# llm-d/llm-d-workload-variant-autoscaler

Hardware: AMD Instinct MI355X
Metric: desired-replica accuracy + SLO-attainment %, Llama-3-8B synthetic QPS ramp (higher is better)
Workload: dtype bf16; 1 GPU; model=meta-llama/Llama-3.1-8B, global_batch=256, seq_len=150, parallelism=dp1, device=AMD Radeon Graphics

## Files before the change

### wva_amd/calibration/model.py

```python
from __future__ import annotations

import math
from dataclasses import dataclass
from typing import List, Optional

import torch

from .. import ops


@dataclass
class LlamaConfig:
    name: str = "llama"
    hidden_size: int = 4096
    intermediate_size: int = 14336
    num_layers: int = 32
    num_q_heads: int = 32
    num_kv_heads: int = 8
    head_dim: int = 128
    vocab_size: int = 128256
    rope_theta: float = 500000.0
    rms_eps: float = 1e-5

    @property
# ... 146 lines not shown
            if self.cache_dtype == torch.bfloat16:
                self.k_cache[layer][:batch, :, :context_len].normal_(0.0, 1.0)
                self.v_cache[layer][:batch, :, :context_len].normal_(0.0, 1.0)
            else:
                shape = self.k_cache[layer][:batch, :, :context_len].shape
                for cache in (self.k_cache, self.v_cache):
                    cache[layer][:batch, :, :context_len] = torch.randn(
                        shape, device=self.device, dtype=torch.bfloat16
                    ).to(self.cache_dtype)

    def _linear(self, x: torch.Tensor, layer, name: str) -> torch.Tensor:
        if self.weights_dtype == "bf16":
            w = getattr(layer, name) if layer is not None else self.lm_head
            return ops.linear(x, w)
        w8, w_scale = (
            getattr(layer, name + "_q") if layer is not None else self.lm_head_q
        )
        if not x.is_cuda:
            return (
                x.float() @ (w8.float() * w_scale[:, None]).t()
            ).to(x.dtype)
        if x.shape[0] <= 64 and x.shape[1] % 128 == 0:
            from .. import ops as _ops

            return _ops._require_ext().skinny_linear_fp8(x, w8, w_scale)
        return (x @ (w8.to(x.dtype) * w_scale[:, None].to(x.dtype)).t())

    @torch.no_grad()
    def decode_step(self, token_ids: torch.Tensor) -> torch.Tensor:
        cfg = self.cfg
        B = token_ids.shape[0]
        positions = self.context_lens[:B].clone()

        ctx = positions + 1
        x = self.embed.index_select(0, token_ids)
        residual: Optional[torch.Tensor] = None

        for li, layer in enumerate(self.layers):
            if residual is None:
                residual = x.clone()
                h = ops.rmsnorm(x, layer.input_norm, None, cfg.rms_eps)
            else:
                h = ops.rmsnorm(x, layer.input_norm, residual, cfg.rms_eps)

            qkv = self._linear(h, layer, "wqkv")
            q = ops.rope_append_kv(
                qkv, self.k_cache[li][:B], self.v_cache[li][:B],
                positions, cfg.num_q_heads, cfg.num_kv_heads, cfg.rope_theta,
            )

            attn = ops.gqa_decode_attn(
                q, self.k_cache[li][:B], self.v_cache[li][:B], ctx, self.scale
            )
            x = self._linear(attn.reshape(B, cfg.q_size), layer, "wo")

            h2 = ops.rmsnorm(x, layer.post_attn_norm, residual, cfg.rms_eps)
            gate_up = self._linear(h2, layer, "w_gate_up")
            act = ops.silu_mul_fused(gate_up)
            x = self._linear(act, layer, "w_down")

        final = ops.rmsnorm(x, self.final_norm, residual, cfg.rms_eps)
        logits = self._linear(final, None, "lm_head")
        self.context_lens[:B] += 1
        return logits

    @torch.no_grad()
    def prefill(self, token_ids: torch.Tensor) -> torch.Tensor:
        cfg = self.cfg
        if self.weights_dtype != "bf16":
            raise NotImplementedError(
                "prefill with fp8 weights is not implemented (the "
                "weight-only fp8 mode targets decode; prefill would "
                "dequantize every layer per pass)"
            )
        B, S = token_ids.shape
        T = B * S
        if S > self.max_seq:
            raise ValueError(f"S={S} exceeds max_seq={self.max_seq}")
        positions = (
            torch.arange(S, device=self.device, dtype=torch.int32)
            .repeat(B)
        )

        x = self.embed.index_select(0, token_ids.reshape(-1))
        residual: Optional[torch.Tensor] = None
# ... 74 lines not shown
```

### wva_amd/calibration/moe_model.py

```python
from __future__ import annotations

import math
from dataclasses import dataclass
from typing import List, Optional

import torch

from .. import ops


@dataclass
class MixtralConfig:
    name: str = "mistralai/Mixtral-8x7B"
    hidden_size: int = 4096
    intermediate_size: int = 14336
    num_layers: int = 32
    num_q_heads: int = 32
    num_kv_heads: int = 8
    head_dim: int = 128
    vocab_size: int = 32000
    rope_theta: float = 1000000.0
    rms_eps: float = 1e-5
    num_experts: int = 8
    top_k: int = 2
# ... 178 lines not shown
        cfg = self.cfg
        B = h2.shape[0]
        E, I = cfg.num_experts, cfg.intermediate_size
        w_full = torch.zeros(B, E, device=h2.device, dtype=h2.dtype)
        w_full.scatter_(1, selected, weights)
        gate_up = ops.linear(h2, layer.w_gate_up_flat)
        act = ops.silu_mul_fused(
            gate_up.reshape(B * E, 2 * I)
        ).reshape(B, E, I)
        y = torch.bmm(act.transpose(0, 1).contiguous(), layer.w_down_t)
        return (y * w_full.t().unsqueeze(-1)).sum(dim=0)

    def _moe_mlp_sparse(self, layer, h2, weights, selected):
        cfg = self.cfg
        out = torch.zeros_like(h2)
        for e in range(cfg.num_experts):
            mask = selected == e
            token_idx, k_idx = mask.nonzero(as_tuple=True)
            if token_idx.numel() == 0:
                continue
            x_e = h2.index_select(0, token_idx)
            gate_up = ops.linear(x_e, layer.w_gate_up[e])
            act = ops.silu_mul_fused(gate_up)
            y = ops.linear(act, layer.w_down[e])
            w_e = weights[token_idx, k_idx].unsqueeze(-1)
            out.index_add_(0, token_idx, (y * w_e).to(out.dtype))
        return out

    @torch.no_grad()
    def decode_step(self, token_ids: torch.Tensor) -> torch.Tensor:
        cfg = self.cfg
        B = token_ids.shape[0]
        positions = self.context_lens[:B].clone()
        ctx = positions + 1

        x = self.embed.index_select(0, token_ids)
        residual: Optional[torch.Tensor] = None

        for li, layer in enumerate(self.layers):
            if residual is None:
                residual = x.clone()
                h = ops.rmsnorm(x, layer.input_norm, None, cfg.rms_eps)
            else:
                h = ops.rmsnorm(x, layer.input_norm, residual, cfg.rms_eps)

            qkv = ops.linear(h, layer.wqkv)
            q = ops.rope_append_kv(
                qkv, self.k_cache[li][:B], self.v_cache[li][:B],
                positions, cfg.num_q_heads, cfg.num_kv_heads, cfg.rope_theta,
            )
            attn = ops.gqa_decode_attn(
                q, self.k_cache[li][:B], self.v_cache[li][:B], ctx, self.scale
            )
            x = ops.linear(attn.reshape(B, cfg.q_size), layer.wo)

            h2 = ops.rmsnorm(x, layer.post_attn_norm, residual, cfg.rms_eps)
            x = self._moe_mlp(layer, h2)

        final = ops.rmsnorm(x, self.final_norm, residual, cfg.rms_eps)
        logits = ops.linear(final, self.lm_head)
        self.context_lens[:B] += 1
        return logits

    @torch.no_grad()
    def prefill(self, token_ids: torch.Tensor) -> torch.Tensor:
        cfg = self.cfg
        B, S = token_ids.shape
        T = B * S
        if S > self.max_seq:
            raise ValueError(f"S={S} exceeds max_seq={self.max_seq}")
        positions = (
            torch.arange(S, device=self.device, dtype=torch.int32).repeat(B)
        )

        x = self.embed.index_select(0, token_ids.reshape(-1))
        residual = None
        causal = None
        if not x.is_cuda:
            causal = torch.full(
                (S, S), float("-inf"), device=self.device, dtype=torch.float32
            ).triu(1)

        for li, layer in enumerate(self.layers):
            if residual is None:
                residual = x.clone()
# ... 60 lines not shown
```

### wva_amd/calibration/tp_model.py

```python
from __future__ import annotations

import math
from typing import List, Optional

import torch
import torch.distributed as dist

from .. import ops
from .model import LlamaConfig


class _TPLayer:
    def __init__(self, cfg: LlamaConfig, shard: "TPShardInfo", device, dtype, gen):
        h, std = cfg.hidden_size, 0.02

        def w(rows, cols):
            return torch.empty(rows, cols, device=device, dtype=dtype).normal_(
                0.0, std, generator=gen
            )

        self.input_norm = torch.ones(h, device=device, dtype=dtype)
        self.post_attn_norm = torch.ones(h, device=device, dtype=dtype)
        self.wqkv = w(shard.q_size + 2 * shard.kv_size, h)
        self.wo = w(h, shard.q_size)
# ... 72 lines not shown
        self.v_cache = [
            torch.zeros_like(self.k_cache[0]) for _ in range(cfg.num_layers)
        ]
        self.context_lens = torch.zeros(
            max_batch, dtype=torch.int32, device=self.device
        )
        self.scale = 1.0 / math.sqrt(cfg.head_dim)

    def _all_reduce(self, x: torch.Tensor) -> torch.Tensor:
        if self.tp > 1:
            dist.all_reduce(x, group=self.group)
        return x

    def reset(self, batch: int, context_len: int) -> None:
        self.context_lens.zero_()
        self.context_lens[:batch] = context_len
        for layer in range(self.cfg.num_layers):
            if self.cache_dtype == torch.bfloat16:
                self.k_cache[layer][:batch, :, :context_len].normal_(0.0, 1.0)
                self.v_cache[layer][:batch, :, :context_len].normal_(0.0, 1.0)
            else:
                shape = self.k_cache[layer][:batch, :, :context_len].shape
                for cache in (self.k_cache, self.v_cache):
                    cache[layer][:batch, :, :context_len] = torch.randn(
                        shape, device=self.device, dtype=torch.bfloat16
                    ).to(self.cache_dtype)

    @torch.no_grad()
    def decode_step(self, token_ids: torch.Tensor) -> torch.Tensor:
        cfg, shard = self.cfg, self.shard
        B = token_ids.shape[0]
        positions = self.context_lens[:B].clone()

        ctx = positions + 1
        x = self.embed.index_select(0, token_ids)
        residual: Optional[torch.Tensor] = None

        for li, layer in enumerate(self.layers):
            if residual is None:
                residual = x.clone()
                h = ops.rmsnorm(x, layer.input_norm, None, cfg.rms_eps)
            else:
                h = ops.rmsnorm(x, layer.input_norm, residual, cfg.rms_eps)

            qkv = ops.linear(h, layer.wqkv)
            q = ops.rope_append_kv(
                qkv, self.k_cache[li][:B], self.v_cache[li][:B],
                positions, shard.num_q_heads, shard.num_kv_heads,
                cfg.rope_theta,
            )
            attn = ops.gqa_decode_attn(
                q, self.k_cache[li][:B], self.v_cache[li][:B], ctx, self.scale
            )
            x = self._all_reduce(ops.linear(attn.reshape(B, shard.q_size), layer.wo))

            h2 = ops.rmsnorm(x, layer.post_attn_norm, residual, cfg.rms_eps)
            gate_up = ops.linear(h2, layer.w_gate_up)
            act = ops.silu_mul_fused(gate_up)
            x = self._all_reduce(ops.linear(act, layer.w_down))

        final = ops.rmsnorm(x, self.final_norm, residual, cfg.rms_eps)
        logits = ops.linear(final, self.lm_head)
        self.context_lens[:B] += 1
        return logits
```

### wva_amd/ops/__init__.py

```python
from __future__ import annotations

import glob
import importlib.util
import math
import os
from typing import Optional

import torch

_HERE = os.path.dirname(os.path.abspath(__file__))
_ext = None
_ext_error: Optional[str] = None


def _try_load_extension():
    global _ext, _ext_error
    if _ext is not None:
        return _ext
    candidates = sorted(glob.glob(os.path.join(_HERE, "_wva_ops*.so")))
    if not candidates:
        _ext_error = (
            f"HIP extension _wva_ops*.so not found in {_HERE}; build it with "
            "`python -m wva_amd.ops.build` (or __graft_entry__.build())"
        )
# ... 228 lines not shown
    idx = torch.arange(B)
    k_cache[idx, :, positions.long()] = k.to(k_cache.dtype)
    v_cache[idx, :, positions.long()] = v.to(v_cache.dtype)
    return q


def silu_mul_fused(gate_up: torch.Tensor) -> torch.Tensor:
    if gate_up.is_cuda:
        return _require_ext().silu_mul_fused(gate_up)
    inter = gate_up.shape[1] // 2
    return silu_mul_ref(gate_up[:, :inter], gate_up[:, inter:]).to(
        gate_up.dtype
    )


def gqa_decode_attn(
    q: torch.Tensor,
    k_cache: torch.Tensor,
    v_cache: torch.Tensor,
    context_lens: torch.Tensor,
    scale: Optional[float] = None,
) -> torch.Tensor:
    if scale is None:
        scale = 1.0 / math.sqrt(q.shape[-1])
    if q.is_cuda:
        return _require_ext().gqa_decode_attn(
            q, k_cache, v_cache, context_lens.to(torch.int32), scale
        )
    return gqa_decode_attn_ref(q, k_cache, v_cache, context_lens, scale).to(
        q.dtype
    )


def moe_route(router_logits: torch.Tensor, top_k: int):
    if router_logits.is_cuda:
        return tuple(
            _require_ext().moe_route(
                router_logits.float().contiguous(), top_k
            )
        )
    return moe_route_ref(router_logits, top_k)


def moe_gate_up_swiglu(
    x: torch.Tensor,
    w_gate_up: torch.Tensor,
    expert_offsets: torch.Tensor,
    sorted_slots: torch.Tensor,
    top_k: int,
) -> torch.Tensor:
    if x.is_cuda:
        return _require_ext().moe_gate_up_swiglu(
            x, w_gate_up, expert_offsets, sorted_slots, top_k
        )
    return moe_gate_up_swiglu_ref(
        x, w_gate_up, expert_offsets, sorted_slots, top_k
    ).to(x.dtype)


def moe_down_combine(
    act_sorted: torch.Tensor,
    w_down: torch.Tensor,
    topk_w: torch.Tensor,
    expert_offsets: torch.Tensor,
    sorted_slots: torch.Tensor,
) -> torch.Tensor:
# ... 71 lines not shown
```

### wva_amd/ops/csrc/attention.hip

```cpp
#include "common.h"

#include <type_traits>

#define HEAD_DIM 128
#define MAX_G 8
#define TILE 64
#define NUM_WAVES 4
#define ROW_DW 66
#define S_ROW 65

template <bool KV_FP8>
using kv_elem_t = std::conditional_t<KV_FP8, fp8_t, bf16>;

__device__ __forceinline__ long ws_row_offset(int b, int kvh, int g, int split,
                                              int num_kv_heads, int G,
                                              int num_splits) {
  return ((((long)b * num_kv_heads + kvh) * G + g) * num_splits + split) *
         (2 + HEAD_DIM);
}

__device__ __forceinline__ long pack8_fp8(const float* v, float inv_scale) {
  unsigned int lo = 0, hi = 0;
  lo = __builtin_amdgcn_cvt_pk_fp8_f32(v[0] * inv_scale, v[1] * inv_scale,
                                       lo, false);
  lo = __builtin_amdgcn_cvt_pk_fp8_f32(v[2] * inv_scale, v[3] * inv_scale,
                                       lo, true);
  hi = __builtin_amdgcn_cvt_pk_fp8_f32(v[4] * inv_scale, v[5] * inv_scale,
                                       hi, false);
  hi = __builtin_amdgcn_cvt_pk_fp8_f32(v[6] * inv_scale, v[7] * inv_scale,
                                       hi, true);
  return (long)(((unsigned long)hi << 32) | lo);
}

struct QFrags {
  bf16x8_frag bf[4];
  long fp8[4];
  float scale;
};

template <bool KV_FP8>
__device__ __forceinline__ QFrags load_q_frags(const bf16* __restrict__ q,
                                               int b, int kvh, int G,
                                               int num_q_heads, int lane,
                                               int wave, int g, int k0,
                                               float* qmax_lds) {
  QFrags qf;
  qf.scale = 1.0f;
#pragma unroll
  for (int kk = 0; kk < 4; ++kk) qf.fp8[kk] = 0;
  float qv[4][8];
#pragma unroll
  for (int kk = 0; kk < 4; ++kk)
#pragma unroll
    for (int i = 0; i < 8; ++i) qv[kk][i] = 0.0f;
  if (g < G) {
    const bf16* qrow = q + ((long)b * num_q_heads + kvh * G + g) * HEAD_DIM;
#pragma unroll
    for (int kk = 0; kk < 4; ++kk) {
      const short* src = reinterpret_cast<const short*>(qrow + 32 * kk + k0);
#pragma unroll
      for (int i = 0; i < 8; ++i) {
        qf.bf[kk][i] = src[i];
        const bf16 bv = *reinterpret_cast<const bf16*>(&src[i]);
        qv[kk][i] = bf2f(bv);
      }
    }
  } else {
#pragma unroll
    for (int kk = 0; kk < 4; ++kk)
#pragma unroll
      for (int i = 0; i < 8; ++i) qf.bf[kk][i] = 0;
  }
  if constexpr (KV_FP8) {
    float amax = 0.0f;
#pragma unroll
    for (int kk = 0; kk < 4; ++kk)
#pragma unroll
      for (int i = 0; i < 8; ++i) amax = fmaxf(amax, fabsf(qv[kk][i]));
    amax = wave_reduce_max(amax);
    if (lane == 0) qmax_lds[wave] = amax;
    __syncthreads();
    float m0 = qmax_lds[0];
#pragma unroll
    for (int w2 = 1; w2 < NUM_WAVES; ++w2) m0 = fmaxf(m0, qmax_lds[w2]);
    qf.scale = fmaxf(m0 / 448.0f, 1e-12f);
    const float inv = 1.0f / qf.scale;
#pragma unroll
    for (int kk = 0; kk < 4; ++kk) qf.fp8[kk] = pack8_fp8(qv[kk], inv);
    __syncthreads();
  }
  return qf;
}

struct SoftmaxStep {
  float p;
  float corr;
};

__device__ __forceinline__ SoftmaxStep online_softmax_step(
    const float* __restrict__ s_row, int tn, int lane, float& m, float& s) {
  const bool live = lane < tn;
  const float score = live ? s_row[lane] : -INFINITY;
  const float tile_max = wave_reduce_max(score);
  const float m_new = fmaxf(m, tile_max);
  const float p = live ? __expf(score - m_new) : 0.0f;
  const float tile_sum = wave_reduce_sum(p);
  const float corr = (m == -INFINITY) ? 0.0f : __expf(m - m_new);
  s = s * corr + tile_sum;
  m = m_new;
  return {p, corr};
}

template <bool KV_FP8>
__global__ __launch_bounds__(256, 2) void gqa_decode_attn_v4_kernel(
    bf16* __restrict__ out,
    float* __restrict__ workspace,
    const bf16* __restrict__ q,
    const void* __restrict__ k_cache,
    const void* __restrict__ v_cache,
    const int* __restrict__ context_lens,
    const int num_q_heads,
    const int num_kv_heads,
    const int max_seq,
    const float scale) {
  const int b = blockIdx.x;
  const int kvh = blockIdx.y;
  const int split = blockIdx.z;
  const int num_splits = gridDim.z;
  const int G = num_q_heads / num_kv_heads;
  const int ctx = context_lens[b];

  const int lane = threadIdx.x & (WAVE_SIZE - 1);
  const int wave = threadIdx.x / WAVE_SIZE;
  const int frag_col = lane % 16;
  const int frag_k0 = 8 * (lane / 16);

  __shared__ float s_smem[MAX_G][S_ROW];
  __shared__ unsigned int v_smem[TILE * ROW_DW];
  __shared__ float p_smem[MAX_G][TILE];
  float* qmax_lds = nullptr;
  if constexpr (KV_FP8) {
    __shared__ float qmax_smem[NUM_WAVES];
    qmax_lds = qmax_smem;
  }

  const QFrags qf = load_q_frags<KV_FP8>(q, b, kvh, G, num_q_heads, lane,
                                         wave, frag_col, frag_k0, qmax_lds);

  const int heads_mine = (G > wave) ? (G - wave + NUM_WAVES - 1) / NUM_WAVES : 0;
  float m[2], s[2], acc[2][2];
#pragma unroll
  for (int j = 0; j < 2; ++j) {
    m[j] = -INFINITY;
    s[j] = 0.0f;
    acc[j][0] = acc[j][1] = 0.0f;
  }

  const long slab_off = ((long)b * num_kv_heads + kvh) * max_seq * HEAD_DIM;
  const auto* k_slab =
      reinterpret_cast<const kv_elem_t<KV_FP8>*>(k_cache) + slab_off;
  const auto* v_slab =
      reinterpret_cast<const kv_elem_t<KV_FP8>*>(v_cache) + slab_off;

  for (int t0 = split * TILE; t0 < ctx; t0 += num_splits * TILE) {
    const int tn = min(TILE, ctx - t0);

    if constexpr (KV_FP8) {
      const int tile_g8 = tn * (HEAD_DIM / 8);
      const fp8_t* v_src = v_slab + (long)t0 * HEAD_DIM;
      for (int idx = wave * WAVE_SIZE + lane; idx < tile_g8;
           idx += NUM_WAVES * WAVE_SIZE) {
        const int row = idx >> 4;
        const int d8 = (idx & 15) * 8;
        const unsigned short* src =
            reinterpret_cast<const unsigned short*>(
                v_src + (long)row * HEAD_DIM + d8);
        unsigned int* dst = &v_smem[row * ROW_DW + d8 / 2];
#pragma unroll
        for (int j = 0; j < 4; ++j) {
          const float2_vt f = unpk2_fp8(src[j]);
// ... 73 lines not shown
        const float p = pg[t];
        a0 = fmaf(p, bf2f(vv.x), a0);
        a1 = fmaf(p, bf2f(vv.y), a1);
      }
      acc[j][0] = a0;
      acc[j][1] = a1;
    }
    __syncthreads();
  }

  if (num_splits == 1) {
    for (int j = 0; j < heads_mine; ++j) {
      const int g = wave + j * NUM_WAVES;
      const float inv = s[j] > 0.0f ? 1.0f / s[j] : 0.0f;
      bf16x2* orow = reinterpret_cast<bf16x2*>(
          out + ((long)b * num_q_heads + kvh * G + g) * HEAD_DIM);
      orow[lane] = bf16x2{f2bf(acc[j][0] * inv), f2bf(acc[j][1] * inv)};
    }
  } else {
    for (int j = 0; j < heads_mine; ++j) {
      const int g = wave + j * NUM_WAVES;
      float* wsp = workspace +
          ws_row_offset(b, kvh, g, split, num_kv_heads, G, num_splits);
      if (lane == 0) {
        wsp[0] = m[j];
        wsp[1] = s[j];
      }
      wsp[2 + 2 * lane] = acc[j][0];
      wsp[2 + 2 * lane + 1] = acc[j][1];
    }
  }
}

template <bool KV_FP8>
__global__ __launch_bounds__(256, 2) void gqa_decode_attn_v5_kernel(
    bf16* __restrict__ out,
    float* __restrict__ workspace,
    const bf16* __restrict__ q,
    const void* __restrict__ k_cache,
    const void* __restrict__ v_cache,
    const int* __restrict__ context_lens,
    const int num_q_heads,
    const int num_kv_heads,
    const int max_seq,
    const float scale) {
  const int b = blockIdx.x;
  const int kvh = blockIdx.y;
  const int split = blockIdx.z;
  const int num_splits = gridDim.z;
  const int G = num_q_heads / num_kv_heads;
  const int ctx = context_lens[b];

  const int lane = threadIdx.x & (WAVE_SIZE - 1);
  const int wave = threadIdx.x / WAVE_SIZE;
  const int frag_col = lane % 16;
  const int frag_k0 = 8 * (lane / 16);

  __shared__ float s_smem[MAX_G][S_ROW];
  __shared__ unsigned int v_smem[TILE * ROW_DW];
  __shared__ float p_smem[MAX_G][TILE];
  __shared__ float corr_smem[MAX_G];
  __shared__ float sum_smem[MAX_G];
  __shared__ float m_smem[MAX_G];
  float* qmax_lds = nullptr;
  if constexpr (KV_FP8) {
    __shared__ float qmax_smem[NUM_WAVES];
    qmax_lds = qmax_smem;
  }

  const QFrags qf = load_q_frags<KV_FP8>(q, b, kvh, G, num_q_heads, lane,
                                         wave, frag_col, frag_k0, qmax_lds);

  const int heads_mine = (G > wave) ? (G - wave + NUM_WAVES - 1) / NUM_WAVES : 0;
  float m[2], s[2];
#pragma unroll
  for (int j = 0; j < 2; ++j) {
    m[j] = -INFINITY;
    s[j] = 0.0f;
  }
  f32x4_frag acc_pv[2] = {f32x4_frag{0.f, 0.f, 0.f, 0.f},
                          f32x4_frag{0.f, 0.f, 0.f, 0.f}};

  const long slab_off = ((long)b * num_kv_heads + kvh) * max_seq * HEAD_DIM;
  const auto* k_slab =
      reinterpret_cast<const kv_elem_t<KV_FP8>*>(k_cache) + slab_off;
  const auto* v_slab =
      reinterpret_cast<const kv_elem_t<KV_FP8>*>(v_cache) + slab_off;

  for (int t0 = split * TILE; t0 < ctx; t0 += num_splits * TILE) {
    const int tn = min(TILE, ctx - t0);

    if constexpr (KV_FP8) {
      const int tile_g8 = tn * (HEAD_DIM / 8);
      const fp8_t* v_src = v_slab + (long)t0 * HEAD_DIM;
      for (int idx = wave * WAVE_SIZE + lane; idx < tile_g8;
           idx += NUM_WAVES * WAVE_SIZE) {
        const int row = idx >> 4;
        const int d8 = (idx & 15) * 8;
        const unsigned short* src =
            reinterpret_cast<const unsigned short*>(
                v_src + (long)row * HEAD_DIM + d8);
        unsigned int* dst = &v_smem[row * ROW_DW + d8 / 2];
#pragma unroll
        for (int j = 0; j < 4; ++j) {
// ... 205 lines not shown
    if (sm_m[w] == -INFINITY) continue;
    const float f = __expf(sm_m[w] - Mg);
    Sg += sm_s[w] * f;
    g0 = fmaf(sm_o[w][2 * lane], f, g0);
    g1 = fmaf(sm_o[w][2 * lane + 1], f, g1);
  }
  const float inv = Sg > 0.0f ? 1.0f / Sg : 0.0f;
  bf16x2* orow = reinterpret_cast<bf16x2*>(
      out + ((long)b * num_q_heads + h) * HEAD_DIM);
  orow[lane] = bf16x2{f2bf(g0 * inv), f2bf(g1 * inv)};
}

extern "C" int gqa_decode_attn_num_splits(int batch, int num_kv_heads,
                                          int max_ctx_hint) {
  const int base = batch * num_kv_heads;
  if (base >= 1792) return 1;
  int splits = 1792 / base;
  static int min_tiles = [] {
    const char* e = getenv("WVA_ATTN_MIN_TILES");
    int v = e ? atoi(e) : 8;
    return v > 0 ? v : 8;
  }();
  int cap = 16;
  if (max_ctx_hint > 0) {
    const int by_work = max_ctx_hint / (min_tiles * TILE);
    if (by_work > cap) cap = by_work;
  }
  if (splits > cap) splits = cap;
  const int max_useful = max_ctx_hint > 0 ? (max_ctx_hint + 2 * TILE - 1) / (2 * TILE) : splits;
  if (splits > max_useful && max_useful >= 1) splits = max_useful;
  return splits < 1 ? 1 : splits;
}

extern "C" void launch_gqa_decode_attn(
    void* out, void* workspace, const void* q, const void* k_cache,
    const void* v_cache, const int* context_lens, int batch, int num_q_heads,
    int num_kv_heads, int max_seq, int num_splits, float scale, int variant,
    int kv_fp8, hipStream_t stream) {
  const auto kernel =
      variant == 5 ? (kv_fp8 ? gqa_decode_attn_v5_kernel<true>
                             : gqa_decode_attn_v5_kernel<false>)
                   : (kv_fp8 ? gqa_decode_attn_v4_kernel<true>
                             : gqa_decode_attn_v4_kernel<false>);
  hipLaunchKernelGGL(kernel, dim3(batch, num_kv_heads, num_splits), dim3(256),
                     0, stream, (bf16*)out, (float*)workspace, (const bf16*)q,
                     k_cache, v_cache, context_lens, num_q_heads, num_kv_heads,
                     max_seq, scale);
  if (num_splits > 1) {
    hipLaunchKernelGGL(gqa_decode_attn_merge_kernel,
                       dim3(batch, num_q_heads), dim3(64 * MERGE_WAVES), 0,
                       stream, (bf16*)out, (const float*)workspace,
                       num_q_heads, num_kv_heads, num_splits);
  }
}
```

### wva_amd/ops/csrc/common.h

```cpp
#pragma once

#include <hip/hip_runtime.h>
#include <hip/hip_bf16.h>

#define WAVE_SIZE 64

using bf16 = __hip_bfloat16;
using bf16x2 = __hip_bfloat162;

__device__ __forceinline__ float bf2f(bf16 v) { return __bfloat162float(v); }
__device__ __forceinline__ bf16 f2bf(float v) { return __float2bfloat16(v); }

typedef __attribute__((ext_vector_type(8))) short bf16x8_frag;
typedef __attribute__((ext_vector_type(4))) float f32x4_frag;
using moe_bf16x8 = bf16x8_frag;
using moe_f32x4 = f32x4_frag;

__device__ __forceinline__ short f2bf_bits(float v) {
  const bf16 b = f2bf(v);
  return *reinterpret_cast<const short*>(&b);
}

__device__ __forceinline__ float wave_reduce_sum(float v) {
#pragma unroll
  for (int offset = 32; offset > 0; offset >>= 1) {
    v += __shfl_xor(v, offset, WAVE_SIZE);
  }
  return v;
}

__device__ __forceinline__ float wave_reduce_max(float v) {
#pragma unroll
  for (int offset = 32; offset > 0; offset >>= 1) {
    v = fmaxf(v, __shfl_xor(v, offset, WAVE_SIZE));
  }
  return v;
}

__device__ __forceinline__ float block_reduce_sum(float v, float* lds) {
  const int lane = threadIdx.x & (WAVE_SIZE - 1);
  const int wave = threadIdx.x / WAVE_SIZE;
  const int num_waves = blockDim.x / WAVE_SIZE;
  v = wave_reduce_sum(v);
  if (lane == 0) lds[wave] = v;
  __syncthreads();
  float out = (lane < num_waves) ? lds[lane] : 0.0f;
  out = wave_reduce_sum(out);
  return __shfl(out, 0, WAVE_SIZE);
}

using fp8_t = unsigned char;
typedef __attribute__((ext_vector_type(2))) float float2_vt;

// ... 18 lines not shown
```

### wva_amd/ops/csrc/ops.cpp

```cpp

#include <torch/extension.h>
#include <hip/hip_runtime.h>
#include <c10/hip/HIPStream.h>

#include <string>

extern "C" void launch_rmsnorm(void* out, void* residual_out,
                               const void* input, const void* residual,
                               const void* weight, float eps, int rows,
                               int hidden, hipStream_t stream);
extern "C" void launch_rope(void* q, void* k, const int* positions, int tokens,
                            int num_q_heads, int num_k_heads, int head_dim,
                            float theta, hipStream_t stream);
extern "C" void launch_silu_mul(void* out, const void* gate, const void* up,
                                long n, hipStream_t stream);
extern "C" void launch_silu_mul_fused(void* out, const void* gate_up,
                                      long rows, long inter,
                                      hipStream_t stream);
extern "C" void launch_rope_append_kv_fp8(const void* qkv, void* q_out,
                                          void* k_cache, void* v_cache,
                                          const int* positions, int batch,
                                          int num_q_heads, int num_kv_heads,
                                          int head_dim, int max_seq,
                                          float theta, hipStream_t stream);
extern "C" void launch_rope_append_kv(const void* qkv, void* q_out,
                                      void* k_cache, void* v_cache,
                                      const int* positions, int batch,
                                      int num_q_heads, int num_kv_heads,
                                      int head_dim, int max_seq, float theta,
                                      hipStream_t stream);
extern "C" int gqa_decode_attn_num_splits(int batch, int num_kv_heads,
                                          int max_ctx_hint);
extern "C" int skinny_gemm_num_splits(int N, int K, int nt);
extern "C" void launch_prefill_attn_ex(void* out, const void* q,
                                       const void* k_cache,
                                       const void* v_cache, int batch,
                                       int seq, int num_q_heads,
                                       int num_kv_heads, int max_seq,
                                       float scale, int kv_fp8,
                                       hipStream_t stream);
extern "C" int skinny_gemm_tile_n(int M);
extern "C" void launch_skinny_gemm(void* c, void* ws, const void* a,
                                   const void* w, int M, int N, int K,
                                   int num_splits, hipStream_t stream);
extern "C" void launch_skinny_gemm_ex(void* c, void* ws, const void* a,
                                      const void* w, const float* w_scale,
                                      int M, int N, int K, int num_splits,
                                      int w_fp8, hipStream_t stream);
extern "C" void launch_gqa_decode_attn(void* out, void* workspace,
                                       const void* q, const void* k_cache,
                                       const void* v_cache,
                                       const int* context_lens, int batch,
                                       int num_q_heads, int num_kv_heads,
                                       int max_seq, int num_splits,
                                       float scale, int variant, int kv_fp8,
                                       hipStream_t stream);

extern "C" int moe_num_m_tiles(int TK, int E);
extern "C" int moe_down_num_splits(int TK, int E, int H, int I);
extern "C" void launch_moe_route(int* topk_idx, float* topk_w,
                                 int* expert_offsets, int* sorted_slots,
                                 const float* logits, int T, int E, int K,
                                 hipStream_t stream);
extern "C" void launch_moe_gate_up_swiglu(void* act, const void* x,
                                          const void* w,
                                          const int* expert_offsets,
                                          const int* sorted_slots, int T,
                                          int E, int top_k, int H, int I,
                                          hipStream_t stream);
extern "C" void launch_moe_down_combine(void* out, float* ws,
                                        const void* act, const void* w,
                                        const float* topk_w,
                                        const int* expert_offsets,
                                        const int* sorted_slots, int T,
                                        int E, int top_k, int H, int I,
                                        int num_splits, hipStream_t stream);

namespace {

hipStream_t current_stream() {
  return c10::hip::getCurrentHIPStream().stream();
}

void check_bf16_contig(const torch::Tensor& t, const char* name) {
  TORCH_CHECK(t.is_cuda(), name, " must be on GPU");
  TORCH_CHECK(t.scalar_type() == torch::kBFloat16, name, " must be bf16");
  TORCH_CHECK(t.is_contiguous(), name, " must be contiguous");
}

// ... 122 lines not shown
  TORCH_CHECK(q.dim() == 3, "q must be [B, Hq, D]");
  TORCH_CHECK(k_cache.dim() == 4,
              "k_cache must be [B, Hk, S, D] (head-major)");
  const int batch = q.size(0);
  const int num_q_heads = q.size(1);
  const int head_dim = q.size(2);
  const int num_kv_heads = k_cache.size(1);
  const int max_seq = k_cache.size(2);
  TORCH_CHECK(head_dim == 128, "head_dim must be 128 (Llama-3 family)");
  TORCH_CHECK(num_q_heads % num_kv_heads == 0, "Hq must divide by Hk");
  const int G = num_q_heads / num_kv_heads;
  TORCH_CHECK(G <= 8, "GQA group size must be <= 8");
  TORCH_CHECK(v_cache.sizes() == k_cache.sizes(), "k/v cache mismatch");
  auto out = torch::empty_like(q);
  const int num_splits =
      gqa_decode_attn_num_splits(batch, num_kv_heads, max_seq);
  if (variant == AttnVariant::Auto) {
    variant = (G >= 8 || num_splits == 1) ? AttnVariant::V5 : AttnVariant::V4;
  }
  torch::Tensor workspace;
  void* ws_ptr = nullptr;
  if (num_splits > 1) {
    workspace = torch::empty(
        {(long)batch * num_kv_heads * G * num_splits * (2 + head_dim)},
        q.options().dtype(torch::kFloat32));
    ws_ptr = workspace.data_ptr();
  }
  launch_gqa_decode_attn(out.data_ptr(), ws_ptr, q.data_ptr(),
                         k_cache.data_ptr(), v_cache.data_ptr(),
                         context_lens.data_ptr<int>(), batch, num_q_heads,
                         num_kv_heads, max_seq, num_splits, (float)scale,
                         variant == AttnVariant::V5 ? 5 : 4, kv_fp8 ? 1 : 0,
                         current_stream());
  return out;
}

torch::Tensor skinny_linear(torch::Tensor x, torch::Tensor w) {
  check_bf16_contig(x, "x");
  check_bf16_contig(w, "w");
  TORCH_CHECK(x.dim() == 2 && w.dim() == 2, "x [M,K], w [N,K]");
  const int M = x.size(0);
  const int K = x.size(1);
  const int N = w.size(0);
  TORCH_CHECK(w.size(1) == K, "K mismatch");
  TORCH_CHECK(M <= 64, "skinny_linear requires M <= 64");
  TORCH_CHECK(K % 128 == 0, "K must be a multiple of 128");
  auto y = torch::empty({M, N}, x.options());
  const int nt = skinny_gemm_tile_n(M);
  const int sk = skinny_gemm_num_splits(N, K, nt);
  torch::Tensor ws;
  void* ws_ptr = nullptr;
  if (sk > 1) {
    ws = torch::empty({(long)sk * M * N},
                      x.options().dtype(torch::kFloat32));
    ws_ptr = ws.data_ptr();
  }
  launch_skinny_gemm(y.data_ptr(), ws_ptr, x.data_ptr(), w.data_ptr(), M, N,
                     K, sk, current_stream());
  return y;
}

torch::Tensor skinny_linear_fp8(torch::Tensor x, torch::Tensor w,
                                torch::Tensor w_scale) {
  check_bf16_contig(x, "x");
  TORCH_CHECK(w.is_cuda() && w.is_contiguous() &&
                  w.scalar_type() == at::kFloat8_e4m3fn,
// ... 157 lines not shown
}

int64_t moe_down_splits(int64_t tokens, int64_t top_k, int64_t num_experts,
                        int64_t hidden, int64_t inter) {
  return moe_down_num_splits((int)(tokens * top_k), (int)num_experts,
                             (int)hidden, (int)inter);
}

}

PYBIND11_MODULE(TORCH_EXTENSION_NAME, m) {
  m.def("rmsnorm", &rmsnorm, "Fused (add-)RMSNorm bf16",
        py::arg("input"), py::arg("weight"), py::arg("residual") = py::none(),
        py::arg("eps") = 1e-5);
  m.def("rope", &rope, "Fused in-place NeoX RoPE on q,k",
        py::arg("q"), py::arg("k"), py::arg("positions"),
        py::arg("theta") = 500000.0);
  m.def("silu_mul", &silu_mul, "Fused SwiGLU silu(gate)*up",
        py::arg("gate"), py::arg("up"));
  m.def("silu_mul_fused", &silu_mul_fused,
        "SwiGLU on the fused [rows, 2*inter] gate_up buffer",
        py::arg("gate_up"));
  m.def("rope_append_kv", &rope_append_kv,
        "RoPE on strided qkv row + KV-cache append; returns contiguous q",
        py::arg("qkv"), py::arg("k_cache"), py::arg("v_cache"),
        py::arg("positions"), py::arg("num_q_heads"), py::arg("num_kv_heads"),
        py::arg("theta") = 500000.0);
  m.def("gqa_decode_attn", &gqa_decode_attn,
        "GQA decode attention over contiguous KV cache; variant pins the "
        "kernel (\"v4\", \"v5\") instead of the measured dispatch (\"auto\")",
        py::arg("q"), py::arg("k_cache"), py::arg("v_cache"),
        py::arg("context_lens"), py::arg("scale"),
        py::arg("variant") = "auto");
  m.def("prefill_attn", &prefill_attn,
        "Causal flash-attention prefill over head-major KV caches",
        py::arg("q"), py::arg("k_cache"), py::arg("v_cache"),
        py::arg("batch"), py::arg("seq"), py::arg("scale"));
  m.def("skinny_linear_fp8", &skinny_linear_fp8,
        "Weight-only fp8 decode GEMM: x[M,K]bf16 @ w[N,K]e4m3^T, M <= 64",
        py::arg("x"), py::arg("w"), py::arg("w_scale"));
  m.def("skinny_linear", &skinny_linear,
        "Weight-streaming decode GEMM: x[M,K] @ w[N,K]^T, M <= 64",
        py::arg("x"), py::arg("w"));
  m.def("moe_route", &moe_route,
        "MoE routing: top-k, softmax weights, expert offsets, sorted slots",
        py::arg("router_logits"), py::arg("top_k"));
  m.def("moe_gate_up_swiglu", &moe_gate_up_swiglu,
        "Grouped gate_up GEMM + SwiGLU over expert-sorted rows",
        py::arg("x"), py::arg("w_gate_up"), py::arg("expert_offsets"),
        py::arg("sorted_slots"), py::arg("top_k"));
  m.def("moe_down_combine", &moe_down_combine,
        "Grouped down GEMM + deterministic top-k combine",
        py::arg("act_sorted"), py::arg("w_down"), py::arg("topk_w"),
        py::arg("expert_offsets"), py::arg("sorted_slots"));
  m.def("moe_down_splits", &moe_down_splits,
        "Split-K factor moe_down_combine uses for these static shapes",
        py::arg("tokens"), py::arg("top_k"), py::arg("num_experts"),
        py::arg("hidden"), py::arg("inter"));
}
```

### wva_amd/ops/csrc/rope.hip

```cpp

#include "common.h"

__device__ __forceinline__ void rotate_pair(
    const bf16* src, bf16* dst, int d, int half, int head_dim, float pos,
    float theta) {
  const float inv_freq = __powf(theta, -2.0f * (float)d / (float)head_dim);
  const float angle = pos * inv_freq;
  float c, s;
  __sincosf(angle, &s, &c);
  const float x1 = bf2f(src[d]);
  const float x2 = bf2f(src[d + half]);
  dst[d] = f2bf(x1 * c - x2 * s);
  dst[d + half] = f2bf(x2 * c + x1 * s);
}

__global__ void rope_kernel(
    bf16* __restrict__ q,
    bf16* __restrict__ k,
    const int* __restrict__ positions,
    const int num_q_heads,
    const int num_k_heads,
    const int head_dim,
    const float theta) {
  const int token = blockIdx.x;
  const float pos = (float)positions[token];
  const int half = head_dim / 2;
  const int total = (num_q_heads + num_k_heads) * half;

  for (int idx = threadIdx.x; idx < total; idx += blockDim.x) {
    const int head = idx / half;
    const int d = idx % half;
    const bool is_q = head < num_q_heads;
    bf16* base = is_q
        ? q + (long)token * num_q_heads * head_dim + (long)head * head_dim
        : k + (long)token * num_k_heads * head_dim +
              (long)(head - num_q_heads) * head_dim;
    rotate_pair(base, base, d, half, head_dim, pos, theta);
  }
}

__global__ void rope_append_kv_kernel(
    const bf16* __restrict__ qkv,
    bf16* __restrict__ q_out,
    bf16* __restrict__ k_cache,
    bf16* __restrict__ v_cache,
    const int* __restrict__ positions,
// ... 34 lines not shown
        v_cache + (((long)b * num_kv_heads + kh) * max_seq + pos_i) * head_dim);
    dst[d2] = vsrc[(long)kh * half + d2];
  }
}

__global__ void rope_append_kv_fp8_kernel(
    const bf16* __restrict__ qkv,
    bf16* __restrict__ q_out,
    fp8_t* __restrict__ k_cache,
    fp8_t* __restrict__ v_cache,
    const int* __restrict__ positions,
    const int num_q_heads,
    const int num_kv_heads,
    const int head_dim,
    const int max_seq,
    const float theta) {
  const int b = blockIdx.x;
  const int pos_i = positions[b];
  const float pos = (float)pos_i;
  const int half = head_dim / 2;
  const long qkv_row = (long)b * (num_q_heads + 2 * num_kv_heads) * head_dim;

  const int rot_total = (num_q_heads + num_kv_heads) * half;
  for (int idx = threadIdx.x; idx < rot_total; idx += blockDim.x) {
    const int head = idx / half;
    const int d = idx % half;
    if (head < num_q_heads) {
      const bf16* src = qkv + qkv_row + (long)head * head_dim;
      bf16* dst = q_out + ((long)b * num_q_heads + head) * head_dim;
      rotate_pair(src, dst, d, half, head_dim, pos, theta);
    } else {
      const int kh = head - num_q_heads;
      const bf16* src = qkv + qkv_row + ((long)num_q_heads + kh) * head_dim;
      const float inv_freq =
          __powf(theta, -2.0f * (float)d / (float)head_dim);
      const float angle = pos * inv_freq;
      float c, s;
      __sincosf(angle, &s, &c);
      const float x1 = bf2f(src[d]);
      const float x2 = bf2f(src[d + half]);
      fp8_t* dst = k_cache +
          (((long)b * num_kv_heads + kh) * max_seq + pos_i) * head_dim;
      dst[d] = f2fp8(x1 * c - x2 * s);
      dst[d + half] = f2fp8(x2 * c + x1 * s);
    }
  }
  const int v_total = num_kv_heads * half;
  const bf16x2* vsrc = reinterpret_cast<const bf16x2*>(
      qkv + qkv_row + (long)(num_q_heads + num_kv_heads) * head_dim);
  for (int idx = threadIdx.x; idx < v_total; idx += blockDim.x) {
    const int kh = idx / half;
    const int d2 = idx % half;
    const bf16x2 v2 = vsrc[(long)kh * half + d2];
    unsigned short* dst = reinterpret_cast<unsigned short*>(
        v_cache + (((long)b * num_kv_heads + kh) * max_seq + pos_i) * head_dim);
    dst[d2] = pk2_fp8(bf2f(v2.x), bf2f(v2.y));
  }
}

extern "C" void launch_rope_append_kv_fp8(
    const void* qkv, void* q_out, void* k_cache, void* v_cache,
    const int* positions, int batch, int num_q_heads, int num_kv_heads,
    int head_dim, int max_seq, float theta, hipStream_t stream) {
  dim3 grid(batch);
  dim3 block(256);
  hipLaunchKernelGGL(rope_append_kv_fp8_kernel, grid, block, 0, stream,
                     (const bf16*)qkv, (bf16*)q_out, (fp8_t*)k_cache,
                     (fp8_t*)v_cache, positions, num_q_heads, num_kv_heads,
                     head_dim, max_seq, theta);
}

extern "C" void launch_rope(
    void* q, void* k, const int* positions, int tokens, int num_q_heads,
    int num_k_heads, int head_dim, float theta, hipStream_t stream) {
  dim3 grid(tokens);
  dim3 block(256);
  hipLaunchKernelGGL(rope_kernel, grid, block, 0, stream, (bf16*)q, (bf16*)k,
// ... 15 lines not shown
```

Before: 91.98 %.

## Fuse RoPE and KV-cache append into the GQA decode attention kernel

Replaces the separate rope_append_kv launch and gqa_decode_attn launch with a single fused kernel. The attention kernel applies RoPE to Q in registers while loading the Q fragments. The split that owns the current tile writes the rotated K and the V row into the cache, then synchronises before reading the tile. This removes one kernel launch per layer, the Q round-trip through global memory and the host-side ctx tensor. In exchange, the owning split does extra work, there is a block-level sync, and the cos/sin values are recomputed in every block.

After: 91.98 %. About the same (+0.0%).

```diff
diff --git a/wva_amd/calibration/model.py b/wva_amd/calibration/model.py
--- a/wva_amd/calibration/model.py
+++ b/wva_amd/calibration/model.py
@@ -202,7 +202,6 @@
         B = token_ids.shape[0]
         positions = self.context_lens[:B].clone()
 
-        ctx = positions + 1
         x = self.embed.index_select(0, token_ids)
         residual: Optional[torch.Tensor] = None
 
@@ -214,13 +213,10 @@
                 h = ops.rmsnorm(x, layer.input_norm, residual, cfg.rms_eps)
 
             qkv = self._linear(h, layer, "wqkv")
-            q = ops.rope_append_kv(
+            attn = ops.rope_gqa_decode_attn(
                 qkv, self.k_cache[li][:B], self.v_cache[li][:B],
                 positions, cfg.num_q_heads, cfg.num_kv_heads, cfg.rope_theta,
-            )
-
-            attn = ops.gqa_decode_attn(
-                q, self.k_cache[li][:B], self.v_cache[li][:B], ctx, self.scale
+                self.scale,
             )
             x = self._linear(attn.reshape(B, cfg.q_size), layer, "wo")
 
diff --git a/wva_amd/calibration/moe_model.py b/wva_amd/calibration/moe_model.py
--- a/wva_amd/calibration/moe_model.py
+++ b/wva_amd/calibration/moe_model.py
@@ -234,7 +234,6 @@
         cfg = self.cfg
         B = token_ids.shape[0]
         positions = self.context_lens[:B].clone()
-        ctx = positions + 1
 
         x = self.embed.index_select(0, token_ids)
         residual: Optional[torch.Tensor] = None
@@ -247,12 +246,10 @@
                 h = ops.rmsnorm(x, layer.input_norm, residual, cfg.rms_eps)
 
             qkv = ops.linear(h, layer.wqkv)
-            q = ops.rope_append_kv(
+            attn = ops.rope_gqa_decode_attn(
                 qkv, self.k_cache[li][:B], self.v_cache[li][:B],
                 positions, cfg.num_q_heads, cfg.num_kv_heads, cfg.rope_theta,
-            )
-            attn = ops.gqa_decode_attn(
-                q, self.k_cache[li][:B], self.v_cache[li][:B], ctx, self.scale
+                self.scale,
             )
             x = ops.linear(attn.reshape(B, cfg.q_size), layer.wo)
 
diff --git a/wva_amd/calibration/tp_model.py b/wva_amd/calibration/tp_model.py
--- a/wva_amd/calibration/tp_model.py
+++ b/wva_amd/calibration/tp_model.py
@@ -128,7 +128,6 @@
         B = token_ids.shape[0]
         positions = self.context_lens[:B].clone()
 
-        ctx = positions + 1
         x = self.embed.index_select(0, token_ids)
         residual: Optional[torch.Tensor] = None
 
@@ -140,13 +139,10 @@
                 h = ops.rmsnorm(x, layer.input_norm, residual, cfg.rms_eps)
 
             qkv = ops.linear(h, layer.wqkv)
-            q = ops.rope_append_kv(
+            attn = ops.rope_gqa_decode_attn(
                 qkv, self.k_cache[li][:B], self.v_cache[li][:B],
                 positions, shard.num_q_heads, shard.num_kv_heads,
-                cfg.rope_theta,
-            )
-            attn = ops.gqa_decode_attn(
-                q, self.k_cache[li][:B], self.v_cache[li][:B], ctx, self.scale
+                cfg.rope_theta, self.scale,
             )
             x = self._all_reduce(ops.linear(attn.reshape(B, shard.q_size), layer.wo))
 
diff --git a/wva_amd/ops/__init__.py b/wva_amd/ops/__init__.py
--- a/wva_amd/ops/__init__.py
+++ b/wva_amd/ops/__init__.py
@@ -284,6 +284,29 @@
     )
 
 
+def rope_gqa_decode_attn(
+    qkv: torch.Tensor,
+    k_cache: torch.Tensor,
+    v_cache: torch.Tensor,
+    positions: torch.Tensor,
+    num_q_heads: int,
+    num_kv_heads: int,
+    theta: float = 500000.0,
+    scale: Optional[float] = None,
+) -> torch.Tensor:
+    if scale is None:
+        scale = 1.0 / math.sqrt(k_cache.shape[-1])
+    if qkv.is_cuda:
+        return _require_ext().rope_gqa_decode_attn(
+            qkv, k_cache, v_cache, positions.to(torch.int32),
+            num_q_heads, num_kv_heads, theta, scale,
+        )
+    q = rope_append_kv(
+        qkv, k_cache, v_cache, positions, num_q_heads, num_kv_heads, theta
+    )
+    return gqa_decode_attn(q, k_cache, v_cache, positions + 1, scale)
+
+
 def moe_route(router_logits: torch.Tensor, top_k: int):
     if router_logits.is_cuda:
         return tuple(
diff --git a/wva_amd/ops/csrc/attention.hip b/wva_amd/ops/csrc/attention.hip
--- a/wva_amd/ops/csrc/attention.hip
+++ b/wva_amd/ops/csrc/attention.hip
@@ -11,6 +11,9 @@
 
 template <bool KV_FP8>
 using kv_elem_t = std::conditional_t<KV_FP8, fp8_t, bf16>;
+
+template <bool FUSED>
+using cache_ptr_t = std::conditional_t<FUSED, void*, const void*>;
 
 __device__ __forceinline__ long ws_row_offset(int b, int kvh, int g, int split,
                                               int num_kv_heads, int G,
@@ -38,12 +41,14 @@
   float scale;
 };
 
-template <bool KV_FP8>
+template <bool KV_FP8, bool FUSED>
 __device__ __forceinline__ QFrags load_q_frags(const bf16* __restrict__ q,
                                                int b, int kvh, int G,
                                                int num_q_heads, int lane,
                                                int wave, int g, int k0,
-                                               float* qmax_lds) {
+                                               float* qmax_lds,
+                                               int num_kv_heads,
+                                               RopeCosSin cs) {
   QFrags qf;
   qf.scale = 1.0f;
 #pragma unroll
@@ -53,7 +58,29 @@
   for (int kk = 0; kk < 4; ++kk)
 #pragma unroll
     for (int i = 0; i < 8; ++i) qv[kk][i] = 0.0f;
-  if (g < G) {
+  if constexpr (FUSED) {
+    const bool live = g < G;
+    const bf16* qrow = q +
+        ((long)b * (num_q_heads + 2 * num_kv_heads) + kvh * G +
+         (live ? g : 0)) * HEAD_DIM;
+#pragma unroll
+    for (int kk = 0; kk < 2; ++kk) {
+#pragma unroll
+      for (int i = 0; i < 8; ++i) {
+        const int d = 32 * kk + k0 + i;
+        const RopeCosSin cs_d = {__shfl(cs.c, d, WAVE_SIZE),
+                                 __shfl(cs.s, d, WAVE_SIZE)};
+        const RopePairBf16 r =
+            rope_apply_bf16(qrow[d], qrow[d + HEAD_DIM / 2], cs_d);
+        qf.bf[kk][i] = live ? *reinterpret_cast<const short*>(&r.lo) : 0;
+        qf.bf[kk + 2][i] = live ? *reinterpret_cast<const short*>(&r.hi) : 0;
+        if (live) {
+          qv[kk][i] = bf2f(r.lo);
+          qv[kk + 2][i] = bf2f(r.hi);
+        }
+      }
+    }
+  } else if (g < G) {
     const bf16* qrow = q + ((long)b * num_q_heads + kvh * G + g) * HEAD_DIM;
 #pragma unroll
     for (int kk = 0; kk < 4; ++kk) {
@@ -90,6 +117,39 @@
     __syncthreads();
   }
   return qf;
+}
+
+template <bool KV_FP8>
+__device__ __forceinline__ void append_kv_row(
+    const bf16* __restrict__ qkv, kv_elem_t<KV_FP8>* k_row,
+    kv_elem_t<KV_FP8>* v_row, int b, int kvh, int num_q_heads,
+    int num_kv_heads, int lane, int wave, RopeCosSin cs) {
+  const bf16* row =
+      qkv + (long)b * (num_q_heads + 2 * num_kv_heads) * HEAD_DIM;
+  constexpr int half = HEAD_DIM / 2;
+  if (wave == 0) {
+    const bf16* src = row + (long)(num_q_heads + kvh) * HEAD_DIM;
+    if constexpr (KV_FP8) {
+      const RopePair r =
+          rope_apply(bf2f(src[lane]), bf2f(src[lane + half]), cs);
+      k_row[lane] = f2fp8(r.lo);
+      k_row[lane + half] = f2fp8(r.hi);
+    } else {
+      const RopePairBf16 r =
+          rope_apply_bf16(src[lane], src[lane + half], cs);
+      k_row[lane] = r.lo;
+      k_row[lane + half] = r.hi;
+    }
+  } else if (wave == 1) {
+    const bf16x2 v2 = reinterpret_cast<const bf16x2*>(
+        row + (long)(num_q_heads + num_kv_heads + kvh) * HEAD_DIM)[lane];
+    if constexpr (KV_FP8) {
+      reinterpret_cast<unsigned short*>(v_row)[lane] =
+          pk2_fp8(bf2f(v2.x), bf2f(v2.y));
+    } else {
+      reinterpret_cast<bf16x2*>(v_row)[lane] = v2;
+    }
+  }
 }
 
 struct SoftmaxStep {
@@ -111,24 +171,26 @@
   return {p, corr};
 }
 
-template <bool KV_FP8>
+template <bool KV_FP8, bool FUSED>
 __global__ __launch_bounds__(256, 2) void gqa_decode_attn_v4_kernel(
     bf16* __restrict__ out,
     float* __restrict__ workspace,
     const bf16* __restrict__ q,
-    const void* __restrict__ k_cache,
-    const void* __restrict__ v_cache,
+    cache_ptr_t<FUSED> __restrict__ k_cache,
+    cache_ptr_t<FUSED> __restrict__ v_cache,
     const int* __restrict__ context_lens,
     const int num_q_heads,
     const int num_kv_heads,
     const int max_seq,
-    const float scale) {
+    const float scale,
+    const float theta) {
   const int b = blockIdx.x;
   const int kvh = blockIdx.y;
   const int split = blockIdx.z;
   const int num_splits = gridDim.z;
   const int G = num_q_heads / num_kv_heads;
-  const int ctx = context_lens[b];
+  const int pos = context_lens[b];
+  const int ctx = !FUSED ? pos : pos < max_seq ? pos + 1 : max_seq;
 
   const int lane = threadIdx.x & (WAVE_SIZE - 1);
   const int wave = threadIdx.x / WAVE_SIZE;
@@ -144,8 +206,28 @@
     qmax_lds = qmax_smem;
   }
 
-  const QFrags qf = load_q_frags<KV_FP8>(q, b, kvh, G, num_q_heads, lane,
-                                         wave, frag_col, frag_k0, qmax_lds);
+  bool owner = false;
+  RopeCosSin cs{};
+  if constexpr (FUSED) {
+    cs = rope_cos_sin(lane, HEAD_DIM, (float)pos, theta);
+    owner = pos >= 0 && pos < max_seq && split == (pos / TILE) % num_splits;
+    if (owner) {
+      const long row_off =
+          (((long)b * num_kv_heads + kvh) * max_seq + pos) * HEAD_DIM;
+      append_kv_row<KV_FP8>(
+          q, reinterpret_cast<kv_elem_t<KV_FP8>*>(k_cache) + row_off,
+          reinterpret_cast<kv_elem_t<KV_FP8>*>(v_cache) + row_off, b, kvh,
+          num_q_heads, num_kv_heads, lane, wave, cs);
+    }
+  }
+
+  const QFrags qf = load_q_frags<KV_FP8, FUSED>(
+      q, b, kvh, G, num_q_heads, lane, wave, frag_col, frag_k0, qmax_lds,
+      num_kv_heads, cs);
+
+  if constexpr (FUSED) {
+    if (owner) __syncthreads();
+  }
 
   const int heads_mine = (G > wave) ? (G - wave + NUM_WAVES - 1) / NUM_WAVES : 0;
   float m[2], s[2], acc[2][2];
@@ -285,24 +367,26 @@
   }
 }
 
-template <bool KV_FP8>
+template <bool KV_FP8, bool FUSED>
 __global__ __launch_bounds__(256, 2) void gqa_decode_attn_v5_kernel(
     bf16* __restrict__ out,
     float* __restrict__ workspace,
     const bf16* __restrict__ q,
-    const void* __restrict__ k_cache,
-    const void* __restrict__ v_cache,
+    cache_ptr_t<FUSED> __restrict__ k_cache,
+    cache_ptr_t<FUSED> __restrict__ v_cache,
     const int* __restrict__ context_lens,
     const int num_q_heads,
     const int num_kv_heads,
     const int max_seq,
-    const float scale) {
+    const float scale,
+    const float theta) {
   const int b = blockIdx.x;
   const int kvh = blockIdx.y;
   const int split = blockIdx.z;
   const int num_splits = gridDim.z;
   const int G = num_q_heads / num_kv_heads;
-  const int ctx = context_lens[b];
+  const int pos = context_lens[b];
+  const int ctx = !FUSED ? pos : pos < max_seq ? pos + 1 : max_seq;
 
   const int lane = threadIdx.x & (WAVE_SIZE - 1);
   const int wave = threadIdx.x / WAVE_SIZE;
@@ -321,8 +405,28 @@
     qmax_lds = qmax_smem;
   }
 
-  const QFrags qf = load_q_frags<KV_FP8>(q, b, kvh, G, num_q_heads, lane,
-                                         wave, frag_col, frag_k0, qmax_lds);
+  bool owner = false;
+  RopeCosSin cs{};
+  if constexpr (FUSED) {
+    cs = rope_cos_sin(lane, HEAD_DIM, (float)pos, theta);
+    owner = pos >= 0 && pos < max_seq && split == (pos / TILE) % num_splits;
+    if (owner) {
+      const long row_off =
+          (((long)b * num_kv_heads + kvh) * max_seq + pos) * HEAD_DIM;
+      append_kv_row<KV_FP8>(
+          q, reinterpret_cast<kv_elem_t<KV_FP8>*>(k_cache) + row_off,
+          reinterpret_cast<kv_elem_t<KV_FP8>*>(v_cache) + row_off, b, kvh,
+          num_q_heads, num_kv_heads, lane, wave, cs);
+    }
+  }
+
+  const QFrags qf = load_q_frags<KV_FP8, FUSED>(
+      q, b, kvh, G, num_q_heads, lane, wave, frag_col, frag_k0, qmax_lds,
+      num_kv_heads, cs);
+
+  if constexpr (FUSED) {
+    if (owner) __syncthreads();
+  }
 
   const int heads_mine = (G > wave) ? (G - wave + NUM_WAVES - 1) / NUM_WAVES : 0;
   float m[2], s[2];
@@ -594,24 +698,51 @@
   return splits < 1 ? 1 : splits;
 }
 
+static void launch_merge(void* out, const void* workspace, int batch,
+                         int num_q_heads, int num_kv_heads, int num_splits,
+                         hipStream_t stream) {
+  hipLaunchKernelGGL(gqa_decode_attn_merge_kernel, dim3(batch, num_q_heads),
+                     dim3(64 * MERGE_WAVES), 0, stream, (bf16*)out,
+                     (const float*)workspace, num_q_heads, num_kv_heads,
+                     num_splits);
+}
+
 extern "C" void launch_gqa_decode_attn(
     void* out, void* workspace, const void* q, const void* k_cache,
     const void* v_cache, const int* context_lens, int batch, int num_q_heads,
     int num_kv_heads, int max_seq, int num_splits, float scale, int variant,
     int kv_fp8, hipStream_t stream) {
   const auto kernel =
-      variant == 5 ? (kv_fp8 ? gqa_decode_attn_v5_kernel<true>
-                             : gqa_decode_attn_v5_kernel<false>)
-                   : (kv_fp8 ? gqa_decode_attn_v4_kernel<true>
-                             : gqa_decode_attn_v4_kernel<false>);
+      variant == 5 ? (kv_fp8 ? gqa_decode_attn_v5_kernel<true, false>
+                             : gqa_decode_attn_v5_kernel<false, false>)
+                   : (kv_fp8 ? gqa_decode_attn_v4_kernel<true, false>
+                             : gqa_decode_attn_v4_kernel<false, false>);
   hipLaunchKernelGGL(kernel, dim3(batch, num_kv_heads, num_splits), dim3(256),
                      0, stream, (bf16*)out, (float*)workspace, (const bf16*)q,
                      k_cache, v_cache, context_lens, num_q_heads, num_kv_heads,
-                     max_seq, scale);
+                     max_seq, scale, 0.0f);
   if (num_splits > 1) {
-    hipLaunchKernelGGL(gqa_decode_attn_merge_kernel,
-                       dim3(batch, num_q_heads), dim3(64 * MERGE_WAVES), 0,
-                       stream, (bf16*)out, (const float*)workspace,
-                       num_q_heads, num_kv_heads, num_splits);
-  }
-}
+    launch_merge(out, workspace, batch, num_q_heads, num_kv_heads, num_splits,
+                 stream);
+  }
+}
+
+extern "C" void launch_rope_gqa_decode_attn(
+    void* out, void* workspace, const void* qkv, void* k_cache, void* v_cache,
+    const int* positions, int batch, int num_q_heads, int num_kv_heads,
+    int max_seq, int num_splits, float theta, float scale, int variant,
+    int kv_fp8, hipStream_t stream) {
+  const auto kernel =
+      variant == 5 ? (kv_fp8 ? gqa_decode_attn_v5_kernel<true, true>
+                             : gqa_decode_attn_v5_kernel<false, true>)
+                   : (kv_fp8 ? gqa_decode_attn_v4_kernel<true, true>
+                             : gqa_decode_attn_v4_kernel<false, true>);
+  hipLaunchKernelGGL(kernel, dim3(batch, num_kv_heads, num_splits), dim3(256),
+                     0, stream, (bf16*)out, (float*)workspace,
+                     (const bf16*)qkv, k_cache, v_cache, positions,
+                     num_q_heads, num_kv_heads, max_seq, scale, theta);
+  if (num_splits > 1) {
+    launch_merge(out, workspace, batch, num_q_heads, num_kv_heads, num_splits,
+                 stream);
+  }
+}
diff --git a/wva_amd/ops/csrc/common.h b/wva_amd/ops/csrc/common.h
--- a/wva_amd/ops/csrc/common.h
+++ b/wva_amd/ops/csrc/common.h
@@ -19,6 +19,55 @@
 __device__ __forceinline__ short f2bf_bits(float v) {
   const bf16 b = f2bf(v);
   return *reinterpret_cast<const short*>(&b);
+}
+
+struct RopeCosSin {
+  float c;
+  float s;
+};
+
+__device__ __forceinline__ RopeCosSin rope_cos_sin(int d, int head_dim,
+                                                   float pos, float theta) {
+  const float inv_freq = __powf(theta, -2.0f * (float)d / (float)head_dim);
+  const float angle = pos * inv_freq;
+  RopeCosSin cs;
+  __sincosf(angle, &cs.s, &cs.c);
+  return cs;
+}
+
+struct RopePair {
+  float lo;
+  float hi;
+};
+
+__device__ __forceinline__ RopePair rope_apply(float x1, float x2,
+                                               RopeCosSin cs) {
+  return {__fmaf_rn(x1, cs.c, -__fmul_rn(x2, cs.s)),
+          __fmaf_rn(x1, cs.s, __fmul_rn(x2, cs.c))};
+}
+
+__device__ __forceinline__ RopePair rope_rotate_f32(float x1, float x2, int d,
+                                                    int head_dim, float pos,
+                                                    float theta) {
+  return rope_apply(x1, x2, rope_cos_sin(d, head_dim, pos, theta));
+}
+
+struct RopePairBf16 {
+  bf16 lo;
+  bf16 hi;
+};
+
+__device__ __forceinline__ RopePairBf16 rope_apply_bf16(bf16 x1, bf16 x2,
+                                                        RopeCosSin cs) {
+  const RopePair r = rope_apply(bf2f(x1), bf2f(x2), cs);
+  return {f2bf(r.lo), f2bf(r.hi)};
+}
+
+__device__ __forceinline__ RopePairBf16 rope_rotate_bf16(bf16 x1, bf16 x2,
+                                                         int d, int head_dim,
+                                                         float pos,
+                                                         float theta) {
+  return rope_apply_bf16(x1, x2, rope_cos_sin(d, head_dim, pos, theta));
 }
 
 __device__ __forceinline__ float wave_reduce_sum(float v) {
diff --git a/wva_amd/ops/csrc/ops.cpp b/wva_amd/ops/csrc/ops.cpp
--- a/wva_amd/ops/csrc/ops.cpp
+++ b/wva_amd/ops/csrc/ops.cpp
@@ -55,6 +55,11 @@
                                        int max_seq, int num_splits,
                                        float scale, int variant, int kv_fp8,
                                        hipStream_t stream);
+extern "C" void launch_rope_gqa_decode_attn(
+    void* out, void* workspace, const void* qkv, void* k_cache, void* v_cache,
+    const int* positions, int batch, int num_q_heads, int num_kv_heads,
+    int max_seq, int num_splits, float theta, float scale, int variant,
+    int kv_fp8, hipStream_t stream);
 
 extern "C" int moe_num_m_tiles(int TK, int E);
 extern "C" int moe_down_num_splits(int TK, int E, int H, int I);
@@ -243,6 +248,60 @@
                          num_kv_heads, max_seq, num_splits, (float)scale,
                          variant == AttnVariant::V5 ? 5 : 4, kv_fp8 ? 1 : 0,
                          current_stream());
+  return out;
+}
+
+torch::Tensor rope_gqa_decode_attn(torch::Tensor qkv, torch::Tensor k_cache,
+                                   torch::Tensor v_cache,
+                                   torch::Tensor positions,
+                                   int64_t num_q_heads, int64_t num_kv_heads,
+                                   double theta, double scale,
+                                   const std::string& variant_name) {
+  AttnVariant variant = parse_attn_variant(variant_name);
+  check_bf16_contig(qkv, "qkv");
+  const bool kv_fp8 = check_cache_contig(k_cache, "k_cache");
+  TORCH_CHECK(check_cache_contig(v_cache, "v_cache") == kv_fp8,
+              "k/v cache dtype mismatch");
+  TORCH_CHECK(qkv.dim() == 2, "qkv must be [B, (Hq+2Hk)*D]");
+  TORCH_CHECK(k_cache.dim() == 4,
+              "k_cache must be [B, Hk, S, D] (head-major)");
+  TORCH_CHECK(v_cache.sizes() == k_cache.sizes(), "k/v cache mismatch");
+  const int batch = qkv.size(0);
+  const int head_dim = k_cache.size(3);
+  const int max_seq = k_cache.size(2);
+  TORCH_CHECK(head_dim == 128, "head_dim must be 128 (Llama-3 family)");
+  TORCH_CHECK(num_q_heads >= 1 && num_kv_heads >= 1, "need Hq, Hk >= 1");
+  TORCH_CHECK(k_cache.size(0) >= batch, "cache holds fewer sequences than qkv");
+  TORCH_CHECK(k_cache.size(1) == num_kv_heads, "Hk mismatch");
+  TORCH_CHECK(qkv.size(1) == (num_q_heads + 2 * num_kv_heads) * head_dim,
+              "qkv width mismatch");
+  TORCH_CHECK(num_q_heads % num_kv_heads == 0, "Hq must divide by Hk");
+  const int G = num_q_heads / num_kv_heads;
+  TORCH_CHECK(G <= 8, "GQA group size must be <= 8");
+  TORCH_CHECK(positions.is_cuda() &&
+                  positions.scalar_type() == torch::kInt32 &&
+                  positions.is_contiguous(),
+              "positions must be contiguous int32 on GPU");
+  TORCH_CHECK(positions.numel() >= batch, "positions must have B entries");
+  auto out = torch::empty({batch, num_q_heads, head_dim}, qkv.options());
+  const int num_splits =
+      gqa_decode_attn_num_splits(batch, num_kv_heads, max_seq);
+  if (variant == AttnVariant::Auto) {
+    variant = (G >= 8 || num_splits == 1) ? AttnVariant::V5 : AttnVariant::V4;
+  }
+  torch::Tensor workspace;
+  void* ws_ptr = nullptr;
+  if (num_splits > 1) {
+    workspace = torch::empty(
+        {(long)batch * num_kv_heads * G * num_splits * (2 + head_dim)},
+        qkv.options().dtype(torch::kFloat32));
+    ws_ptr = workspace.data_ptr();
+  }
+  launch_rope_gqa_decode_attn(
+      out.data_ptr(), ws_ptr, qkv.data_ptr(), k_cache.data_ptr(),
+      v_cache.data_ptr(), positions.data_ptr<int>(), batch, (int)num_q_heads,
+      (int)num_kv_heads, max_seq, num_splits, (float)theta, (float)scale,
+      variant == AttnVariant::V5 ? 5 : 4, kv_fp8 ? 1 : 0, current_stream());
   return out;
 }
 
@@ -466,6 +525,12 @@
         py::arg("q"), py::arg("k_cache"), py::arg("v_cache"),
         py::arg("context_lens"), py::arg("scale"),
         py::arg("variant") = "auto");
+  m.def("rope_gqa_decode_attn", &rope_gqa_decode_attn,
+        "rope_append_kv + gqa_decode_attn at positions + 1 in one attention "
+        "launch; appends to the caches in place and returns out [B, Hq, 128]",
+        py::arg("qkv"), py::arg("k_cache"), py::arg("v_cache"),
+        py::arg("positions"), py::arg("num_q_heads"), py::arg("num_kv_heads"),
+        py::arg("theta"), py::arg("scale"), py::arg("variant") = "auto");
   m.def("prefill_attn", &prefill_attn,
         "Causal flash-attention prefill over head-major KV caches",
         py::arg("q"), py::arg("k_cache"), py::arg("v_cache"),
diff --git a/wva_amd/ops/csrc/rope.hip b/wva_amd/ops/csrc/rope.hip
--- a/wva_amd/ops/csrc/rope.hip
+++ b/wva_amd/ops/csrc/rope.hip
@@ -4,14 +4,10 @@
 __device__ __forceinline__ void rotate_pair(
     const bf16* src, bf16* dst, int d, int half, int head_dim, float pos,
     float theta) {
-  const float inv_freq = __powf(theta, -2.0f * (float)d / (float)head_dim);
-  const float angle = pos * inv_freq;
-  float c, s;
-  __sincosf(angle, &s, &c);
-  const float x1 = bf2f(src[d]);
-  const float x2 = bf2f(src[d + half]);
-  dst[d] = f2bf(x1 * c - x2 * s);
-  dst[d + half] = f2bf(x2 * c + x1 * s);
+  const RopePairBf16 r =
+      rope_rotate_bf16(src[d], src[d + half], d, head_dim, pos, theta);
+  dst[d] = r.lo;
+  dst[d + half] = r.hi;
 }
 
 __global__ void rope_kernel(
@@ -112,17 +108,12 @@
     } else {
       const int kh = head - num_q_heads;
       const bf16* src = qkv + qkv_row + ((long)num_q_heads + kh) * head_dim;
-      const float inv_freq =
-          __powf(theta, -2.0f * (float)d / (float)head_dim);
-      const float angle = pos * inv_freq;
-      float c, s;
-      __sincosf(angle, &s, &c);
-      const float x1 = bf2f(src[d]);
-      const float x2 = bf2f(src[d + half]);
+      const RopePair r = rope_rotate_f32(bf2f(src[d]), bf2f(src[d + half]),
+                                         d, head_dim, pos, theta);
       fp8_t* dst = k_cache +
           (((long)b * num_kv_heads + kh) * max_seq + pos_i) * head_dim;
-      dst[d] = f2fp8(x1 * c - x2 * s);
-      dst[d + half] = f2fp8(x2 * c + x1 * s);
+      dst[d] = f2fp8(r.lo);
+      dst[d + half] = f2fp8(r.hi);
     }
   }
   const int v_total = num_kv_heads * half;
```
